# TaceoLabs/co-snarks

Hardware: AMD Instinct MI355X
Metric: BN254 G1 MSM points/sec (higher is better)
Workload: dtype i32x9 29-bit-limb lazy Montgomery, i64 accumulate (BN254 Fq 254-bit); 1 GPU; BN254 G1 Pippenger MSM, uniform scalars / known-dlog points, 2^20 points per GPU (BASELINE config 2); points_total=1048576, points_per_gpu=1048576, split=single GPU, exchange_mode=none, rccl_ranks_seen=0, spinup_steps=190

## Files before the change

### co-snarks_amd/csrc/msm_impl.hpp

```cpp
#pragma once
#include <stdlib.h>
#include <string.h>

#include <algorithm>
#include <type_traits>
#include <vector>

#include "common.hpp"
#include "curve.hpp"
#include "curve_lazy.hpp"
#include "curve_quad.hpp"
#include "curve_pair.hpp"
#include "host_fp64.hpp"
#include "msm_digits.hpp"
#include "msm_plan.hpp"
#include "msm_sort.hpp"
#include "msm_sort_wide.hpp"


namespace csh {

struct Bn254G1Cfg { using Fq = Bn254Fq;   using Fr = Bn254Fr; static constexpr bool LAZY = true;  using L = Fq29s; static constexpr bool INLINE_ADD = true; static constexpr bool PAIR = false; };
struct Bn254G2Cfg { using Fq = Bn254Fq2;  using Fr = Bn254Fr; static constexpr bool LAZY = true;  using L = Fq29s2; static constexpr bool INLINE_ADD = true; static constexpr bool PAIR = true; static constexpr bool PAIR_ACC_DEFAULT = false; using LP = Fp2Pair<Fq29s>; };
struct Bls381G1Cfg { using Fq = Bls381Fq;  using Fr = Bls381Fr; static constexpr bool LAZY = true;  using L = Fq28s; static constexpr bool INLINE_ADD = true; static constexpr bool PAIR = false; };
// ... 458 lines not shown
}

template <class Cfg, bool FUSED>
__global__ __launch_bounds__(RED_BLK) void k_msm_reduce_pair(MsmParams p, const LazyPt<Cfg>* __restrict__ dense, LazyPt<Cfg>* segres,
                                                             const uint32_t* __restrict__ start, const LazyPt<Cfg>* __restrict__ partial) {
  using L = typename Cfg::LP;
  const int w = blockIdx.y;
  const int role = pair_role();
  const uint32_t k = blockIdx.x * (RED_BLK / 2) + (threadIdx.x >> 1);
  if (k >= p.S) return;
  const uint32_t per = (p.NB + p.S - 1) / p.S;
  const uint32_t t0 = 1 + k * per;
  uint32_t t1 = t0 + per;
  if (t1 > p.NB + 1) t1 = p.NB + 1;
  XYZZLazy<L> running = XYZZLazy<L>::inf(), acc = XYZZLazy<L>::inf();
  uint32_t prev_b = 0;
  if (t0 < t1) {
    const LazyPt<Cfg>* dw = dense + (size_t)w * (p.NB + 1);
    const uint32_t* st = FUSED ? start + (size_t)w * (p.NB + 2) : nullptr;
    const LazyPt<Cfg>* pw = FUSED ? partial + (size_t)w * p.tmax : nullptr;
    for (uint32_t t = t1; t-- > t0;) {
      XYZZLazy<L> pt;
      if constexpr (FUSED) {
        pt = pbucket_merged<Cfg>(lane_len(p, w), st, pw, dw, t, role);
        if (pt.empty) continue;
      } else {
        if (dw[t].empty) continue;
        pt = pair_load(&dw[t], role);
      }
      uint32_t gap = prev_b ? prev_b - t : 0;
      if (gap) {
        if (gap <= 4) {
          while (gap--) lazy_add_inl<L>(acc, running);
        } else {
          const XYZZLazy<L> m = lazy_mul_small<L, true>(running, gap);
          lazy_add_inl<L>(acc, m);
        }
      }
      lazy_add_inl<L>(running, pt);
      prev_b = t;
    }
    if (prev_b) {
      const XYZZLazy<L> m = lazy_mul_small<L, true>(running, prev_b);
      lazy_add_inl<L>(acc, m);
    }
  }
  pair_store(&segres[(size_t)w * p.S + k], role, acc);
}

template <class Cfg>
__global__ __launch_bounds__(256) void k_msm_fold_tree(const LazyPt<Cfg>* __restrict__ in, uint32_t stride_in, uint32_t count,
                                                       LazyPt<Cfg>* out, uint32_t stride_out, XYZZ<typename Cfg::Fq>* win_out) {
  using L = typename Cfg::L;
  using Fq = typename Cfg::Fq;
  __shared__ XYZZLazy<L> sh[32];
  const int w = blockIdx.y;
  const int role = threadIdx.x & 3, q = threadIdx.x >> 2;
  const LazyPt<Cfg>* a = in + (size_t)w * stride_in;
  const uint32_t i0 = blockIdx.x * 128 + q, i1 = i0 + 64;
  QPt<L> x = i0 < count ? qpt_load<L>(&a[i0], role) : qpt_inf<L>();
  if (i1 < count) qadd<L>(x, qpt_load<L>(&a[i1], role), role);
  quad_block_tree<L>(x, sh, q, 64, role);
  if (q == 0) {
    if (win_out) {
      static_assert(sizeof(XYZZ<Fq>) == 4 * sizeof(Fq), "XYZZ members must be contiguous");
      (&win_out[w].x)[role] = x.empty ? Fq::zero() : x.v.to_fp();
    } else {
      qpt_store<L>(&out[(size_t)w * stride_out + blockIdx.x], role, x);
    }
  }
}

template <class Cfg>
__global__ __launch_bounds__(256) void k_bases_repack(Affine<typename Cfg::Fq>* pts, size_t n) {
  if constexpr (Cfg::LAZY) {
    using L = typename Cfg::L;
    for (size_t i = blockIdx.x * (size_t)256 + threadIdx.x; i < n; i += (size_t)gridDim.x * 256) {
      Affine<typename Cfg::Fq> p = pts[i];
      if (p.is_inf()) continue;
      p.x = L::repack_for_storage(p.x);
      p.y = L::repack_for_storage(p.y);
      pts[i] = p;
    }
  }
}

template <class Cfg>
__global__ void k_msm_gather_windows(const LazyPt<Cfg>* segres, uint32_t stride, int W, XYZZ<typename Cfg::Fq>* out) {
  const int w = threadIdx.x;
  if (w < W) out[w] = lazy_to_xyzz<typename Cfg::L, typename Cfg::Fq>(segres[(size_t)w * stride]);
}

extern thread_local float tl_msm_timing[6];
extern thread_local uint32_t tl_msm_params[4];
inline void msm_record_params(const MsmParams& srt) {
  tl_msm_params[0] = (uint32_t)srt.c;
  tl_msm_params[1] = (uint32_t)srt.W;
  tl_msm_params[2] = srt.L;
  tl_msm_params[3] = srt.S;
}

struct Events {
  std::vector<hipEvent_t> ev;
  Events() = default;
  Events(const Events&) = delete;
  Events& operator=(const Events&) = delete;
  ~Events() {
    for (hipEvent_t e : ev) (void)hipEventDestroy(e);
  }
  int create(size_t count, unsigned flags) {
    ev.reserve(ev.size() + count);
    for (size_t i = 0; i < count; ++i) {
      hipEvent_t e;
      CSH_HIP(hipEventCreateWithFlags(&e, flags));
      ev.push_back(e);
    }
    return CSH_OK;
  }
  hipEvent_t operator[](size_t i) const { return ev[i]; }
};

struct PartialHeader {
  uint32_t magic, c, W, wide;
  uint32_t pad[4];
};
constexpr uint32_t PARTIAL_MAGIC = 0x4d534d50u;


struct SortOut {
  uint32_t *start, *nlanes, *sorted;
};

inline bool msm_sort_is_wide(const MsmParams& p) { return p.c > 16 && p.W == 1 && p.remap_n != 0; }
template <class Fr>
constexpr int fr_id_of() {
  return std::is_same<Fr, Bls381Fr>::value ? 1 : (std::is_same<Fr, Bn254Fq>::value ? 2 : (std::is_same<Fr, Bls377Fr>::value ? 3 : 0));
}

struct SortStageBufs {
  SortBuffers sb;
  bool two_level;
};
inline SortBuffers sort_group_view(const MsmParams& p, const SortBuffers& b, int w0) {
  const size_t len = (size_t)p.NB + 2, n = p.n;
  SortBuffers g = b;
  g.hist += len * w0;
  g.start += len * w0;
  g.nlanes += w0;
  g.sorted += n * w0;
  g.dig += n * w0;
  g.blkcnt += (size_t)p.NB * p.CH * w0;
  if (g.inter) g.inter += n * w0;
  if (g.part_cnt) g.part_cnt += (size_t)(p.NB / 256) * p.CH * w0;
  return g;
}
inline SortStageBufs sort_take(const MsmParams& p, Arena& ar) {
  const size_t len = (size_t)p.NB + 2, n = p.n;
  SortStageBufs s;
  s.sb.hist = ar.take<uint32_t>(len * p.W);
  s.sb.start = ar.take<uint32_t>(len * p.W);
  s.sb.nlanes = ar.take<uint32_t>(MAX_WINDOWS);
  s.sb.sorted = ar.take<uint32_t>(n * p.W);
  s.sb.dig = ar.take<uint16_t>(n * p.W);
  s.sb.blkcnt = ar.take<uint32_t>((size_t)p.NB * p.CH * p.W);
  s.two_level = msm_sort_two_level(p);
  s.sb.inter = s.two_level ? ar.take<uint64_t>(n * p.W) : nullptr;
  s.sb.part_cnt = s.two_level ? ar.take<uint32_t>((size_t)(p.NB / 256) * p.CH * p.W) : nullptr;
  return s;
}
inline size_t msm_sort_bytes(const MsmParams& p, const MsmParams& pdig) {
  if (msm_sort_is_wide(p)) return msm_sort_wide_bytes(p, pdig);
  Arena sizing;
  sort_take(p, sizing);
  return sizing.off;
}
template <class Fr>
int msm_sort_prepare(const MsmParams& p, const MsmParams& pdig, const uint64_t* scalars_dev, hipStream_t st, Arena& ar, SortStageBufs* out) {
  *out = sort_take(p, ar);
  const int g1 = grid_for(pdig.n, MSM_BLK, 65536);
  hipLaunchKernelGGL(k_msm_digits<Fr>, dim3(g1), dim3(MSM_BLK), 0, st, reinterpret_cast<const Fr*>(scalars_dev), pdig, const_cast<uint16_t*>(out->sb.dig));
  return CSH_OK;
}
template <class Fr>
int msm_sort_stage(const MsmParams& p, const MsmParams& pdig, const uint64_t* scalars_dev, hipStream_t st, Arena& ar, SortOut* out, hipEvent_t* ev) {
  if (msm_sort_is_wide(p)) return msm_sort_wide_launch(fr_id_of<Fr>(), p, pdig, scalars_dev, st, ar, &out->start, &out->nlanes, &out->sorted, ev);
  SortStageBufs ss;
  CSH_TRY(msm_sort_prepare<Fr>(p, pdig, scalars_dev, st, ar, &ss));
  CSH_TRY(msm_sort_launch(p, ss.sb, st, ev));
  *out = SortOut{ss.sb.start, ss.sb.nlanes, ss.sb.sorted};
  return CSH_OK;
}

template <class Cfg>
struct BucketBufs {
  LazyPt<Cfg>*partial, *segres, *dense, *fold_a, *fold_b;
  uint32_t* giant;
  uint32_t* big;
  LazyPt<Cfg>* gscratch;
  uint32_t fold_n1, max_lanes, max_giant, giant_blocks;
};
constexpr int MAX_GROUPS = 8;
template <class Cfg>
BucketBufs<Cfg> bucket_take(const MsmParams& p, Arena& ar) {
  BucketBufs<Cfg> b;
  b.max_lanes = (uint32_t)(((size_t)p.n + p.L - 1) / p.L);
  b.max_giant = (uint32_t)(((uint64_t)b.max_lanes * p.W) / MERGE_CAP + 1);
  b.giant_blocks = b.max_giant < 1024 ? b.max_giant : 1024;
  b.partial = ar.take<LazyPt<Cfg>>((size_t)p.tmax * p.W);
  b.segres = ar.take<LazyPt<Cfg>>((size_t)p.S * p.W);
  b.dense = ar.take<LazyPt<Cfg>>((size_t)(p.NB + 1) * p.W);
  b.giant = ar.take<uint32_t>((2 * (size_t)b.max_giant + 2) * MAX_GROUPS);
  b.big = ar.take<uint32_t>((size_t)2 * GIANT_BIG_CAP * MAX_GROUPS);
  b.gscratch = ar.take<LazyPt<Cfg>>((size_t)GIANT_BIG_CAP * GIANT_SLICES * MAX_GROUPS);
  b.fold_n1 = (p.S + 127) / 128;
  b.fold_a = ar.take<LazyPt<Cfg>>((size_t)b.fold_n1 * p.W);
  b.fold_b = ar.take<LazyPt<Cfg>>((size_t)b.fold_n1 * p.W);
  return b;
}
template <class Cfg>
size_t msm_bucket_bytes(const MsmParams* pp) {
  Arena sizing;
  bucket_take<Cfg>(*pp, sizing);
  return sizing.off;
}

template <class Cfg>
struct BucketSumViews {
  const uint32_t *start, *nlanes, *sorted;
  LazyPt<Cfg>*partial, *dense;
  uint32_t *giant, *big;
  LazyPt<Cfg>* gscratch;
};
template <class Cfg>
int bucket_sums_launch(const Affine<typename Cfg::Fq>* bases, const MsmParams& p, const BucketSumViews<Cfg>& v, uint32_t max_lanes, uint32_t giant_blocks, int nw,
                       bool pair, bool fused, hipStream_t st, hipEvent_t* ev) {
  {
    const int tb = tune().acc_blk.load(std::memory_order_relaxed);
    const int blk = (tb == 64 || tb == 128) ? tb : ACC_BLK;
    if constexpr (Cfg::PAIR) {
      if (pair) {
        const dim3 ag((2 * max_lanes + blk - 1) / blk, nw), ab(blk);
        hipLaunchKernelGGL(k_msm_accum_pair<Cfg>, ag, ab, 0, st, bases, p, v.start, v.nlanes, v.sorted, v.partial, v.giant);
      }
    }
    if (!(Cfg::PAIR && pair)) {
      const dim3 ag((max_lanes + blk - 1) / blk, nw), ab(blk);
      hipLaunchKernelGGL(k_msm_accum<Cfg>, ag, ab, 0, st, bases, p, v.start, v.nlanes, v.sorted, v.partial, v.giant);
    }
  }
  if (ev) CSH_HIP(hipEventRecord(ev[4], st));
  if (fused)
    hipLaunchKernelGGL(k_msm_mark_giant<Cfg>, dim3((p.NB + 255) / 256, nw), dim3(256), 0, st, p, v.start, v.giant, v.giant + 2, v.big);
  else
    hipLaunchKernelGGL(k_msm_merge<Cfg>, dim3((p.NB + MERGE_Q - 1) / MERGE_Q, nw), dim3(MERGE_BLK), 0, st, p, v.start, v.partial, v.dense, v.giant, v.giant + 2, v.big);
  hipLaunchKernelGGL(k_msm_giant_slices<Cfg>, dim3(GIANT_SLICES, GIANT_ROWS), dim3(256), 0, st, p, v.start, v.partial, v.giant, v.big, v.gscratch);
  hipLaunchKernelGGL(k_msm_merge_giant<Cfg>, dim3(giant_blocks), dim3(256), 0, st, p, v.start, v.partial, v.dense, v.giant, v.giant + 2, v.big, v.gscratch);
  return CSH_OK;
}

template <class Cfg>
int bucket_group(const void* points, const MsmParams& p_all, const SortOut& so, const BucketBufs<Cfg>& bb, int w0, int nw, int group, hipStream_t st,
                 void* win_out_dev, hipEvent_t* ev) {
  using Fq = typename Cfg::Fq;
  MsmParams p = p_all;
  p.wide = p_all.wide > w0 ? p_all.wide - w0 : 0;
  const size_t len = (size_t)p.NB + 2;
  const uint32_t* start = so.start + len * w0;
  LazyPt<Cfg>* partial = bb.partial + (size_t)p.tmax * w0;
  LazyPt<Cfg>* segres = bb.segres + (size_t)p.S * w0;
  LazyPt<Cfg>* dense = bb.dense + (size_t)(p.NB + 1) * w0;
  LazyPt<Cfg>* fold_a = bb.fold_a + (size_t)bb.fold_n1 * w0;
  LazyPt<Cfg>* fold_b = bb.fold_b + (size_t)bb.fold_n1 * w0;
  const BucketSumViews<Cfg> views{start, so.nlanes + w0, so.sorted + (size_t)p.n * w0, partial, dense, bb.giant + (2 * (size_t)bb.max_giant + 2) * group,
                                  bb.big + (size_t)2 * GIANT_BIG_CAP * group, bb.gscratch + (size_t)GIANT_BIG_CAP * GIANT_SLICES * group};
  const int variant = tune().msm_variant.load(std::memory_order_relaxed);
  bool pair = false;
  if constexpr (Cfg::PAIR) pair = Cfg::PAIR_ACC_DEFAULT != ((variant & 2) != 0);
  int form;
  if constexpr (Cfg::PAIR) form = (variant & 1) ? 1 : ((variant & 4) ? 0 : 2);
  else form = (variant & 1) ? 0 : 1;
  const bool fused = form != 0 && (variant & 16) != 0;
  CSH_TRY((bucket_sums_launch<Cfg>(reinterpret_cast<const Affine<Fq>*>(points), p, views, bb.max_lanes, bb.giant_blocks, nw, pair, fused, st, ev)));
  MsmParams pr = p;
  if (form == 1) {
    pr.S = std::min(p.S, reduce_segments(p.NB, p.W, 4));
    if (fused) hipLaunchKernelGGL((k_msm_reduce<Cfg, true>), dim3((pr.S + 63) / 64, nw), dim3(256), 0, st, pr, dense, segres, start, partial);
    else hipLaunchKernelGGL((k_msm_reduce<Cfg, false>), dim3((pr.S + 63) / 64, nw), dim3(256), 0, st, pr, dense, segres, start, partial);
  } else if (form == 2) {
    pr.S = std::min(p.S, reduce_segments(p.NB, p.W, 2));
    if constexpr (Cfg::PAIR) {
      if (fused) hipLaunchKernelGGL((k_msm_reduce_pair<Cfg, true>), dim3((pr.S + RED_BLK / 2 - 1) / (RED_BLK / 2), nw), dim3(RED_BLK), 0, st, pr, dense, segres, start, partial);
      else hipLaunchKernelGGL((k_msm_reduce_pair<Cfg, false>), dim3((pr.S + RED_BLK / 2 - 1) / (RED_BLK / 2), nw), dim3(RED_BLK), 0, st, pr, dense, segres, start, partial);
    }
  } else {
    hipLaunchKernelGGL(k_msm_reduce_serial<Cfg>, dim3((pr.S + RED_BLK - 1) / RED_BLK, nw), dim3(RED_BLK), 0, st, pr, dense, segres);
  }
  const LazyPt<Cfg>* cur = segres;
  uint32_t cur_n = pr.S, cur_stride = pr.S;
  LazyPt<Cfg>* nxt = fold_a;
  XYZZ<Fq>* win_out = reinterpret_cast<XYZZ<Fq>*>(win_out_dev) + w0;
  bool exported = false;
  while (cur_n > 1) {
    const uint32_t out_n = (cur_n + 127) / 128;
    exported = out_n == 1;
    hipLaunchKernelGGL(k_msm_fold_tree<Cfg>, dim3(out_n, nw), dim3(256), 0, st, cur, cur_stride, cur_n, nxt, bb.fold_n1,
                       exported ? win_out : (XYZZ<Fq>*)nullptr);
    cur = nxt;
    cur_n = out_n;
    cur_stride = bb.fold_n1;
    nxt = nxt == fold_a ? fold_b : fold_a;
  }
  if (!exported)
    hipLaunchKernelGGL(k_msm_gather_windows<Cfg>, dim3(1), dim3(MAX_WINDOWS), 0, st, cur, cur_stride, nw, win_out);
  CSH_HIP(hipGetLastError());
  return CSH_OK;
}

template <class Cfg>
int msm_bucket_stage(const void* points, const MsmParams* pp, const SortOut* so, hipStream_t st, Arena* arp, void* win_out_dev, hipEvent_t* ev) {
  const MsmParams& p = *pp;
// ... 459 lines not shown
```

### co-snarks_amd/csrc/msm_sort.hip

```cpp
#include <stdlib.h>

#include "msm_sort.hpp"

namespace csh {

__device__ __forceinline__ uint32_t entry_id(const MsmParams& p, size_t i) {
  if (p.remap_n == 0) return (uint32_t)i;
  const uint32_t f = (uint32_t)i;
  const uint32_t w = f / p.remap_n;
  return w * p.remap_stride + p.remap_off + (f - w * p.remap_n);
}

__global__ __launch_bounds__(SORT_BLK) void k_msm_hist_lds(MsmParams p, const uint16_t* __restrict__ dig, uint32_t* __restrict__ blkcnt,
                                                            uint32_t* __restrict__ part_cnt ) {
  extern __shared__ uint32_t lds_cnt[];
  const uint32_t ch = blockIdx.x, w = blockIdx.y;
  for (uint32_t b = threadIdx.x; b < p.NB; b += SORT_BLK) lds_cnt[b] = 0;
  __syncthreads();
  const size_t lo = (size_t)ch * p.chunk_len;
  size_t hi = lo + p.chunk_len;
  if (hi > p.n) hi = p.n;
  const uint16_t* d = dig + (size_t)w * p.n;
  for (size_t i0 = lo; i0 < hi; i0 += 4 * SORT_BLK) {
    uint32_t code[4];
#pragma unroll
    for (int k = 0; k < 4; ++k) {
      const size_t i = i0 + (size_t)k * SORT_BLK + threadIdx.x;
      code[k] = i < hi ? (uint32_t)d[i] : DIG_ZERO;
    }
#pragma unroll
    for (int k = 0; k < 4; ++k) (void)lds_slot(lds_cnt, code[k] & 0x7fffu, code[k] != DIG_ZERO);
  }
  __syncthreads();
  uint32_t* out = blkcnt + ((size_t)w * p.CH + ch) * p.NB;
  for (uint32_t b = threadIdx.x; b < p.NB; b += SORT_BLK) out[b] = lds_cnt[b];
  if (part_cnt) {
    const uint32_t P = p.NB / 256;
    const int lane = threadIdx.x & 63;
    for (uint32_t part = threadIdx.x >> 6; part < P; part += SORT_BLK / 64) {
      const uint32_t* c = lds_cnt + part * 256;
      uint32_t v = c[lane] + c[lane + 64] + c[lane + 128] + c[lane + 192];
#pragma unroll
      for (int d = 32; d >= 1; d >>= 1) v += (uint32_t)__shfl_xor((int)v, d);
      if (lane == 0) part_cnt[((size_t)w * p.CH + ch) * P + part] = v;
    }
  }
}

__global__ __launch_bounds__(256) void k_msm_colscan(MsmParams p, uint32_t* __restrict__ blkcnt, uint32_t* __restrict__ hist) {
  const uint32_t w = blockIdx.y;
  const uint32_t b = blockIdx.x * 256 + threadIdx.x;
  if (b >= p.NB) return;
  uint32_t acc = 0;
  uint32_t* col = blkcnt + (size_t)w * p.CH * p.NB + b;
  for (uint32_t ch0 = 0; ch0 < p.CH; ch0 += 8) {
    uint32_t t[8];
#pragma unroll
    for (uint32_t j = 0; j < 8; ++j) t[j] = ch0 + j < p.CH ? col[(size_t)(ch0 + j) * p.NB] : 0u;
#pragma unroll
    for (uint32_t j = 0; j < 8; ++j) {
      if (ch0 + j < p.CH) col[(size_t)(ch0 + j) * p.NB] = acc;
      acc += t[j];
    }
  }
  hist[(size_t)w * (p.NB + 2) + b + 1] = acc;
  if (b == 0) {
    hist[(size_t)w * (p.NB + 2)] = 0;
    hist[(size_t)w * (p.NB + 2) + p.NB + 1] = 0;
  }
}

__global__ __launch_bounds__(1024) void k_msm_scan(MsmParams p, uint32_t* hist, uint32_t* start, uint32_t* nlanes) {
  extern __shared__ uint32_t sc_lds[];
  const int w = blockIdx.x;
  const uint32_t len = p.NB + 2;
  uint32_t* h = hist + (size_t)w * len;
  uint32_t* st = start + (size_t)w * len;
  uint32_t* wave_tot = sc_lds + len;
  for (uint32_t b = threadIdx.x; b < len; b += 1024) sc_lds[b] = h[b];
  __syncthreads();
  const uint32_t per = (len + 1023) / 1024;
  const uint32_t b0 = threadIdx.x * per;
  uint32_t cnt = 0;
  for (uint32_t k = 0; k < per; ++k) {
    const uint32_t b = b0 + k;
    if (b < len) cnt += sc_lds[b];
  }
  uint32_t total;
  uint32_t run_c = block_excl_scan<16>(cnt, wave_tot, &total);
  for (uint32_t k = 0; k < per; ++k) {
    const uint32_t b = b0 + k;
    if (b < len) {
      const uint32_t cv = sc_lds[b];
      sc_lds[b] = run_c;
      run_c += cv;
    }
  }
  __syncthreads();
  for (uint32_t b = threadIdx.x; b < len; b += 1024) {
    st[b] = sc_lds[b];
    h[b] = sc_lds[b];
  }
  if (threadIdx.x == 0) nlanes[w] = (total + lane_len(p, w) - 1) / lane_len(p, w);
}

__global__ __launch_bounds__(SORT_BLK) void k_msm_scatter_lds(MsmParams p, const uint16_t* __restrict__ dig,
                                                               const uint32_t* __restrict__ start, const uint32_t* __restrict__ blkcnt,
                                                               uint32_t* __restrict__ sorted) {
  extern __shared__ uint32_t lds_cur[];
  const uint32_t ch = blockIdx.x, w = blockIdx.y;
  const uint32_t* st = start + (size_t)w * (p.NB + 2) + 1;
  const uint32_t* pre = blkcnt + ((size_t)w * p.CH + ch) * p.NB;
  for (uint32_t b = threadIdx.x; b < p.NB; b += SORT_BLK) lds_cur[b] = st[b] + pre[b];
  __syncthreads();
  const size_t lo = (size_t)ch * p.chunk_len;
  size_t hi = lo + p.chunk_len;
  if (hi > p.n) hi = p.n;
  const uint16_t* d = dig + (size_t)w * p.n;
  uint32_t* so = sorted + (size_t)w * p.n;
  for (size_t i0 = lo; i0 < hi; i0 += SORT_BLK) {
    const size_t i = i0 + threadIdx.x;
    uint32_t code = DIG_ZERO;
    if (i < hi) code = d[i];
    const bool valid = code != DIG_ZERO;
    const uint32_t pos = lds_slot(lds_cur, code & 0x7fffu, valid);
    if (valid) so[pos] = entry_id(p, i) | ((code >> 15) << 31);
  }
}


constexpr uint32_t PART_BUCKETS = 256;
constexpr uint32_t PART_LB = 8;
static_assert(PART_BUCKETS == 1u << PART_LB, "the record format's low key must hold a partition's bucket index");

__global__ __launch_bounds__(256) void k_msm_part_offsets(MsmParams p, const uint32_t* __restrict__ start, uint32_t* part_cnt) {
  const uint32_t P = p.NB / PART_BUCKETS;
  const uint32_t part = blockIdx.x * 256 + threadIdx.x, w = blockIdx.y;
  if (part >= P) return;
  uint32_t run = start[(size_t)w * (p.NB + 2) + (size_t)part * PART_BUCKETS + 1];
  uint32_t* col = part_cnt + (size_t)w * p.CH * P + part;
  for (uint32_t ch0 = 0; ch0 < p.CH; ch0 += 8) {
    uint32_t c[8];
#pragma unroll
    for (uint32_t j = 0; j < 8; ++j) c[j] = ch0 + j < p.CH ? col[(size_t)(ch0 + j) * P] : 0u;
#pragma unroll
    for (uint32_t j = 0; j < 8; ++j) {
      if (ch0 + j < p.CH) col[(size_t)(ch0 + j) * P] = run;
      run += c[j];
    }
  }
}

#ifndef CSH_L1_WPE
#define CSH_L1_WPE 8
#endif
#if CSH_L1_WPE > 0
#define CSH_L1_OCC __attribute__((amdgpu_waves_per_eu(CSH_L1_WPE)))
#else
#define CSH_L1_OCC
#endif
constexpr int L1_EPT = 8;
constexpr int L1_TILE = L1_EPT * SORT_BLK;
constexpr uint32_t MAXP = 128;
template <int REC>
__global__ __launch_bounds__(SORT_BLK) CSH_L1_OCC void k_msm_scatter_l1(MsmParams p, const uint16_t* __restrict__ dig, const uint32_t* __restrict__ part_off,
                                                             void* __restrict__ inter) {
  __shared__ uint32_t gcur[MAXP];
  __shared__ uint32_t cnt[MAXP];
  __shared__ uint32_t toff[MAXP];
  __shared__ uint32_t wsum[2];
  __shared__ uint32_t pay[L1_TILE];
  __shared__ uint8_t slo[L1_TILE];
  __shared__ uint8_t sbin[L1_TILE];
  const uint32_t ch = blockIdx.x, w = blockIdx.y, tid = threadIdx.x;
  const uint32_t P = p.NB / PART_BUCKETS;
  if (tid < MAXP) {
    gcur[tid] = tid < P ? part_off[((size_t)w * p.CH + ch) * P + tid] : 0;
    cnt[tid] = 0;
  }
  __syncthreads();
  const size_t lo = (size_t)ch * p.chunk_len;
  size_t hi = lo + p.chunk_len;
  if (hi > p.n) hi = p.n;
  const uint16_t* d = dig + (size_t)w * p.n;
  SortRec<REC>* out = reinterpret_cast<SortRec<REC>*>(inter) + (size_t)w * p.n;
  for (size_t t0 = lo; t0 < hi; t0 += L1_TILE) {
    uint32_t code[L1_EPT], rank[L1_EPT];
#pragma unroll
    for (int k = 0; k < L1_EPT; ++k) {
      const size_t i = t0 + (size_t)k * SORT_BLK + tid;
      code[k] = i < hi ? (uint32_t)__builtin_nontemporal_load(d + i) : DIG_ZERO;
    }
#pragma unroll
    for (int k = 0; k < L1_EPT; ++k) rank[k] = lds_slot(cnt, (code[k] & 0x7fffu) / PART_BUCKETS, code[k] != DIG_ZERO);
    __syncthreads();
    const uint32_t v = tid < MAXP ? cnt[tid] : 0;
    uint32_t tile_n;
    const uint32_t excl = block_excl_scan<MAXP / 64, SORT_BLK / 64>(v, wsum, &tile_n);
    if (tid < MAXP) toff[tid] = excl;
    __syncthreads();
#pragma unroll
    for (int k = 0; k < L1_EPT; ++k) {
      if (code[k] != DIG_ZERO) {
        const uint32_t b0 = code[k] & 0x7fffu;
        const uint32_t slot = toff[b0 / PART_BUCKETS] + rank[k];
        pay[slot] = entry_id(p, t0 + (size_t)k * SORT_BLK + tid) | ((code[k] >> 15) << 31);
        slo[slot] = (uint8_t)(b0 % PART_BUCKETS);
        sbin[slot] = (uint8_t)(b0 / PART_BUCKETS);
      }
    }
    __syncthreads();
#pragma unroll
    for (int k = 0; k < L1_EPT; ++k) {
      const uint32_t sl = k * SORT_BLK + tid;
      if (sl < tile_n) {
        const uint32_t bin = sbin[sl];
        out[gcur[bin] + (sl - toff[bin])] = rec_pack<REC>(pay[sl], slo[sl], PART_LB);
      }
    }
    __syncthreads();
    if (tid < MAXP) {
      gcur[tid] += v;
      cnt[tid] = 0;
    }
    __syncthreads();
  }
}

struct L2Lds {
  uint32_t obase[PART_BUCKETS];
  uint32_t cnt[PART_BUCKETS];
  uint32_t toff[PART_BUCKETS];
  uint32_t wsum[4];
  uint32_t pay[L2_TILE];
  uint8_t sbin[L2_TILE];
};
struct L2OwnRuns {
  __device__ void reserve(uint32_t*, uint32_t, uint32_t) const {}
  __device__ void advance(uint32_t* obase, uint32_t b, uint32_t v) const { obase[b] += v; }
};
struct L2SharedRuns {
  uint32_t* cur;
  __device__ void reserve(uint32_t* obase, uint32_t b, uint32_t v) const { obase[b] = v ? atomicAdd(&cur[b], v) : 0u; }
  __device__ void advance(uint32_t*, uint32_t, uint32_t) const {}
};
template <int REC, class Runs>
__device__ __forceinline__ void l2_sort_slice(L2Lds& s, const Runs runs, const SortRec<REC>* __restrict__ in, uint32_t lo, uint32_t hi,
                                              uint32_t* __restrict__ so) {
  const uint32_t tid = threadIdx.x;
  for (uint32_t t0 = lo; t0 < hi; t0 += L2_TILE) {
    SortRec<REC> e[L2_EPT];
    uint32_t rank[L2_EPT];
    l2_load_rank<REC>(in, t0, hi, PART_LB, s.cnt, e, rank);
    __syncthreads();
    uint32_t v = 0, total;
    if (tid < PART_BUCKETS) {
      v = s.cnt[tid];
      runs.reserve(s.obase, tid, v);
    }
    const uint32_t excl = block_excl_scan<PART_BUCKETS / 64, SORT_BLK / 64>(v, s.wsum, &total);
    if (tid < PART_BUCKETS) s.toff[tid] = excl;
    __syncthreads();
#pragma unroll
    for (int k = 0; k < L2_EPT; ++k) {
      if (t0 + k * SORT_BLK + tid < hi) {
        const uint32_t bin = rec_low<REC>(e[k], PART_LB);
        const uint32_t slot = s.toff[bin] + rank[k];
        s.pay[slot] = rec_entry<REC>(e[k], PART_LB);
        s.sbin[slot] = (uint8_t)bin;
      }
    }
    __syncthreads();
    const uint32_t tile_n = hi - t0 < (uint32_t)L2_TILE ? hi - t0 : (uint32_t)L2_TILE;
#pragma unroll
    for (int k = 0; k < L2_EPT; ++k) {
      const uint32_t sl = k * SORT_BLK + tid;
      if (sl < tile_n) {
        const uint32_t bin = s.sbin[sl];
        so[s.obase[bin] + (sl - s.toff[bin])] = s.pay[sl];
      }
    }
    __syncthreads();
    if (tid < PART_BUCKETS) {
      runs.advance(s.obase, tid, v);
      s.cnt[tid] = 0;
    }
    __syncthreads();
  }
}

template <int REC>
__global__ __launch_bounds__(SORT_BLK) void k_msm_scatter_l2(MsmParams p, const uint32_t* __restrict__ start, const void* __restrict__ inter,
                                                             uint32_t* __restrict__ sorted) {
  __shared__ L2Lds s;
  const uint32_t part = blockIdx.x, w = blockIdx.y, tid = threadIdx.x;
  const uint32_t* st = start + (size_t)w * (p.NB + 2) + (size_t)part * PART_BUCKETS + 1;
  if (tid < PART_BUCKETS) {
    s.obase[tid] = st[tid];
    s.cnt[tid] = 0;
  }
  __syncthreads();
  l2_sort_slice<REC>(s, L2OwnRuns{}, reinterpret_cast<const SortRec<REC>*>(inter) + (size_t)w * p.n, st[0], st[PART_BUCKETS],
                     sorted + (size_t)w * p.n);
}

template <int REC>
__global__ __launch_bounds__(SORT_BLK) void k_msm_scatter_l2t(MsmParams p, const uint32_t* __restrict__ start, uint32_t* __restrict__ cursor,
                                                              const void* __restrict__ inter, uint32_t* __restrict__ sorted) {
  __shared__ L2Lds s;
  __shared__ uint32_t job[3];
  const uint32_t x = blockIdx.x, w = blockIdx.y, tid = threadIdx.x;
  const uint32_t P = p.NB / PART_BUCKETS;
  const uint32_t* stw = start + (size_t)w * (p.NB + 2);
  {
    uint32_t lo_p = 0, hi_p = 0, nb = 0, total;
    if (tid < P) {
      lo_p = stw[(size_t)tid * PART_BUCKETS + 1];
      hi_p = stw[(size_t)(tid + 1) * PART_BUCKETS + 1];
      const uint32_t c = hi_p - lo_p;
      nb = c ? (c + L2_TILE / 2) / L2_TILE : 0;
      if (c && nb == 0) nb = 1;
    }
    if (tid == 0) job[0] = 0xffffffffu;
    const uint32_t pre = block_excl_scan<MAXP / 64, SORT_BLK / 64>(nb, s.wsum, &total);
    if (nb && x >= pre && x < pre + nb) {
      const uint32_t c = hi_p - lo_p, slice = (c + nb - 1) / nb, j = x - pre;
      uint32_t a = lo_p + j * slice, b = a + slice;
      if (b > hi_p) b = hi_p;
      if (a > hi_p) a = hi_p;
      job[0] = tid;
      job[1] = a;
      job[2] = b;
    }
    __syncthreads();
  }
  const uint32_t part = job[0];
  if (part == 0xffffffffu) return;
  if (tid < PART_BUCKETS) s.cnt[tid] = 0;
  __syncthreads();
  l2_sort_slice<REC>(s, L2SharedRuns{cursor + (size_t)w * (p.NB + 2) + (size_t)part * PART_BUCKETS + 1},
                     reinterpret_cast<const SortRec<REC>*>(inter) + (size_t)w * p.n, job[1], job[2], sorted + (size_t)w * p.n);
}

bool msm_sort_two_level(const MsmParams& p) {
  if (p.NB < 4 * PART_BUCKETS) return false;
  if (const int f = tune().sort_two_level.load(std::memory_order_relaxed); f >= 0) return f != 0;
  return p.n >= (1u << 20);
}

SortPath msm_sort_path(const MsmParams& p) {
  SortPath s{msm_sort_two_level(p), false, false};
  if (!s.two_level) return s;
  const uint64_t max_id = p.remap_n ? (uint64_t)(p.n / p.remap_n) * p.remap_stride : (uint64_t)p.n;
  const int variant = tune().msm_variant.load(std::memory_order_relaxed);
  s.rec4 = (variant & 8) == 0 && max_id <= (1u << (31 - PART_LB));
  s.per_partition = (variant & 32) != 0;
  return s;
}

template <int REC>
static void launch_two_level(const MsmParams& p, const SortBuffers& b, bool per_partition, hipStream_t st) {
  const uint32_t nparts = p.NB / PART_BUCKETS;
  hipLaunchKernelGGL(k_msm_scatter_l1<REC>, dim3(p.CH, p.W), dim3(SORT_BLK), 0, st, p, b.dig, b.part_cnt, (void*)b.inter);
  if (per_partition) {
    hipLaunchKernelGGL(k_msm_scatter_l2<REC>, dim3(nparts, p.W), dim3(SORT_BLK), 0, st, p, b.start, (const void*)b.inter, b.sorted);
  } else {
    const uint32_t l2_blocks = (uint32_t)(p.n / L2_TILE) + nparts + 1;
    hipLaunchKernelGGL(k_msm_scatter_l2t<REC>, dim3(l2_blocks, p.W), dim3(SORT_BLK), 0, st, p, b.start, b.hist, (const void*)b.inter, b.sorted);
  }
}

int msm_sort_launch(const MsmParams& p, const SortBuffers& b, hipStream_t st, hipEvent_t* ev) {
  const SortPath path = msm_sort_path(p);
  const bool two_level = path.two_level;
  const size_t sort_lds = sizeof(uint32_t) * p.NB;
  if (sort_lds > 48 * 1024) {
    CSH_TRY(raise_lds_limit((const void*)k_msm_hist_lds, 128 * 1024));
    CSH_TRY(raise_lds_limit((const void*)k_msm_scatter_lds, 128 * 1024));
  }
  hipLaunchKernelGGL(k_msm_hist_lds, dim3(p.CH, p.W), dim3(SORT_BLK), sort_lds, st, p, b.dig, b.blkcnt, two_level ? b.part_cnt : nullptr);
  hipLaunchKernelGGL(k_msm_colscan, dim3((p.NB + 255) / 256, p.W), dim3(256), 0, st, p, b.blkcnt, b.hist);
  if (ev) CSH_HIP(hipEventRecord(ev[1], st));
  {
    const size_t scan_lds = sizeof(uint32_t) * ((size_t)p.NB + 2 + 16);
    if (scan_lds > 48 * 1024) CSH_TRY(raise_lds_limit((const void*)k_msm_scan, 136 * 1024));
    hipLaunchKernelGGL(k_msm_scan, dim3(p.W), dim3(1024), scan_lds, st, p, b.hist, b.start, b.nlanes);
  }
  if (ev) CSH_HIP(hipEventRecord(ev[2], st));
  if (two_level) {
    hipLaunchKernelGGL(k_msm_part_offsets, dim3((p.NB / PART_BUCKETS + 255) / 256, p.W), dim3(256), 0, st, p, b.start, b.part_cnt);
    path.rec4 ? launch_two_level<1>(p, b, path.per_partition, st) : launch_two_level<0>(p, b, path.per_partition, st);
  } else {
    hipLaunchKernelGGL(k_msm_scatter_lds, dim3(p.CH, p.W), dim3(SORT_BLK), sort_lds, st, p, b.dig, b.start, b.blkcnt, b.sorted);
  }
  if (ev) CSH_HIP(hipEventRecord(ev[3], st));
  return CSH_OK;
}

}
```

### co-snarks_amd/csrc/msm_sort.hpp

```cpp
#pragma once
#include <type_traits>

#include "common.hpp"

namespace csh {

struct MsmParams {
  uint32_t n;
  int c;
  int W;
  uint32_t NB;
  uint32_t L;
  uint32_t tmax;
  uint32_t S;
  int mont;
  uint32_t CH;
  uint32_t chunk_len;
  uint32_t remap_n, remap_stride, remap_off;
  uint32_t dig_g, dig_wp;
  int wide;
  uint32_t Ln;
};
__host__ __device__ inline uint32_t lane_len(const MsmParams& p, int w) { return w >= p.wide ? p.Ln : p.L; }

constexpr uint32_t DIG_ZERO = 0xFFFFu;
constexpr int MAX_WINDOWS = 128;

struct SortBuffers {
  uint32_t* hist;
  uint32_t* start;
  uint32_t* nlanes;
  uint32_t* sorted;
  const uint16_t* dig;
  uint32_t* blkcnt;
  uint64_t* inter;
  uint32_t* part_cnt;
};

#if defined(__HIPCC__)
__device__ __forceinline__ uint32_t lds_slot(uint32_t* counter, uint32_t b, bool valid) {
  uint32_t slot = 0;
  bool todo = valid;
  for (int round = 0; round < 4; ++round) {
    const unsigned long long act = __ballot(todo);
    if (!act) return slot;
    const int leader = __ffsll((long long)act) - 1;
    const uint32_t lb = (uint32_t)__shfl((int)b, leader);
    const unsigned long long grp = __ballot(todo && b == lb);
    const int cnt = __popcll(grp);
    if (cnt < 8) break;
    uint32_t base = 0;
    const int lane = threadIdx.x & 63;
    if (lane == leader) base = atomicAdd(&counter[lb], (uint32_t)cnt);
    base = (uint32_t)__shfl((int)base, leader);
    if (todo && b == lb) {
      slot = base + (uint32_t)__popcll(grp & ((1ull << lane) - 1ull));
      todo = false;
    }
  }
  if (todo) slot = atomicAdd(&counter[b], 1u);
  return slot;
}

__device__ __forceinline__ uint32_t wave_incl_scan(uint32_t v) {
  const int lane = threadIdx.x & 63;
#pragma unroll
  for (int d = 1; d < 64; d <<= 1) {
    const uint32_t up = (uint32_t)__shfl_up((int)v, d);
    if (lane >= d) v += up;
  }
  return v;
}

template <int NW, int BLOCK_WAVES = NW>
__device__ __forceinline__ uint32_t block_excl_scan(uint32_t v, uint32_t* wsum, uint32_t* total) {
  const int lane = threadIdx.x & 63, wv = threadIdx.x >> 6;
  uint32_t incl = 0;
  if (BLOCK_WAVES == NW || wv < NW) {
    incl = wave_incl_scan(v);
    if (lane == 63) wsum[wv] = incl;
  }
  __syncthreads();
  uint32_t base = 0, tot = 0;
#pragma unroll
  for (int i = 0; i < NW; ++i) {
    const uint32_t t = wsum[i];
    if (i < wv) base += t;
    tot += t;
  }
  *total = tot;
  return base + incl - v;
}

template <int REC>
using SortRec = typename std::conditional<REC != 0, uint32_t, uint64_t>::type;
template <int REC>
__device__ __forceinline__ SortRec<REC> rec_pack(uint32_t entry, uint32_t low, uint32_t lb) {
  if constexpr (REC == 1) {
    const uint32_t idb = 31 - lb;
    return (entry & ((1u << idb) - 1)) | ((entry >> 31) << idb) | (low << (idb + 1));
  } else {
    return (uint64_t)entry | ((uint64_t)low << 32);
  }
}
template <int REC>
__device__ __forceinline__ uint32_t rec_low(SortRec<REC> e, uint32_t lb) {
  if constexpr (REC == 1) return e >> (32 - lb);
  else return (uint32_t)(e >> 32);
}
template <int REC>
__device__ __forceinline__ uint32_t rec_entry(SortRec<REC> e, uint32_t lb) {
  if constexpr (REC == 1) {
    const uint32_t idb = 31 - lb;
    return (e & ((1u << idb) - 1)) | (((e >> idb) & 1u) << 31);
  } else {
    return (uint32_t)e;
  }
}

constexpr int SORT_BLK = 1024;
constexpr int L2_EPT = 8;
constexpr int L2_TILE = L2_EPT * SORT_BLK;
template <int REC>
__device__ __forceinline__ void l2_load_rank(const SortRec<REC>* __restrict__ in, uint32_t t0, uint32_t hi, uint32_t lb, uint32_t* cnt,
                                             SortRec<REC>* e, uint32_t* rank) {
#pragma unroll
  for (int k = 0; k < L2_EPT; ++k) {
    const uint32_t i = t0 + k * SORT_BLK + threadIdx.x;
    e[k] = i < hi ? __builtin_nontemporal_load(in + i) : 0;
  }
#pragma unroll
  for (int k = 0; k < L2_EPT; ++k) rank[k] = lds_slot(cnt, rec_low<REC>(e[k], lb), t0 + k * SORT_BLK + threadIdx.x < hi);
}
#endif

bool msm_sort_two_level(const MsmParams& p);
struct SortPath {
  bool two_level;
  bool rec4;
  bool per_partition;
};
SortPath msm_sort_path(const MsmParams& p);
int msm_sort_launch(const MsmParams& p, const SortBuffers& b, hipStream_t st, hipEvent_t* ev);

}
```

Measured before the change: 663.9 million points/s.

## Precompute L2 sort jobs, prefetch L1 digit tiles, skip unused colscan prefix writes

Several sort-stage changes land together. The per-block job assignment that every L2 scatter block recomputed with a scan is moved into k_msm_part_offsets, which writes a job table once per window. The L1 scatter now does vectorized 4-digit loads, packs two ranks per register, and prefetches the next tile while the current one is scattered, and it merges the cursor updates to drop two barriers per tile. Colscan skips writing per-chunk prefixes when the two-level path does not use them. The cost is extra job-table memory, a single-block-per-window part_offsets kernel, and the prefetch registers may reduce occupancy.

```diff
diff --git a/co-snarks_amd/csrc/msm_impl.hpp b/co-snarks_amd/csrc/msm_impl.hpp
--- a/co-snarks_amd/csrc/msm_impl.hpp
+++ b/co-snarks_amd/csrc/msm_impl.hpp
@@ -634,6 +634,7 @@
   g.blkcnt += (size_t)p.NB * p.CH * w0;
   if (g.inter) g.inter += n * w0;
   if (g.part_cnt) g.part_cnt += (size_t)(p.NB / 256) * p.CH * w0;
+  if (g.l2_jobs) g.l2_jobs += (size_t)4 * msm_l2_jobs(p) * w0;
   return g;
 }
 inline SortStageBufs sort_take(const MsmParams& p, Arena& ar) {
@@ -648,6 +649,7 @@
   s.two_level = msm_sort_two_level(p);
   s.sb.inter = s.two_level ? ar.take<uint64_t>(n * p.W) : nullptr;
   s.sb.part_cnt = s.two_level ? ar.take<uint32_t>((size_t)(p.NB / 256) * p.CH * p.W) : nullptr;
+  s.sb.l2_jobs = s.two_level ? ar.take<uint32_t>((size_t)4 * msm_l2_jobs(p) * p.W) : nullptr;
   return s;
 }
 inline size_t msm_sort_bytes(const MsmParams& p, const MsmParams& pdig) {
diff --git a/co-snarks_amd/csrc/msm_sort.hip b/co-snarks_amd/csrc/msm_sort.hip
--- a/co-snarks_amd/csrc/msm_sort.hip
+++ b/co-snarks_amd/csrc/msm_sort.hip
@@ -47,6 +47,7 @@
   }
 }
 
+template <bool PREFIX>
 __global__ __launch_bounds__(256) void k_msm_colscan(MsmParams p, uint32_t* __restrict__ blkcnt, uint32_t* __restrict__ hist) {
   const uint32_t w = blockIdx.y;
   const uint32_t b = blockIdx.x * 256 + threadIdx.x;
@@ -59,7 +60,7 @@
     for (uint32_t j = 0; j < 8; ++j) t[j] = ch0 + j < p.CH ? col[(size_t)(ch0 + j) * p.NB] : 0u;
 #pragma unroll
     for (uint32_t j = 0; j < 8; ++j) {
-      if (ch0 + j < p.CH) col[(size_t)(ch0 + j) * p.NB] = acc;
+      if (PREFIX && ch0 + j < p.CH) col[(size_t)(ch0 + j) * p.NB] = acc;
       acc += t[j];
     }
   }
@@ -133,21 +134,60 @@
 constexpr uint32_t PART_LB = 8;
 static_assert(PART_BUCKETS == 1u << PART_LB, "the record format's low key must hold a partition's bucket index");
 
-__global__ __launch_bounds__(256) void k_msm_part_offsets(MsmParams p, const uint32_t* __restrict__ start, uint32_t* part_cnt) {
+constexpr uint32_t MAXP = 128;
+constexpr uint32_t L2_NO_JOB = 0xffffffffu;
+__global__ __launch_bounds__(256) void k_msm_part_offsets(MsmParams p, const uint32_t* __restrict__ start, uint32_t* part_cnt, uint4* __restrict__ jobs,
+                                                          uint32_t njobs) {
+  __shared__ uint32_t s_pre[MAXP + 1], s_lo[MAXP], s_hi[MAXP], s_wsum[4];
   const uint32_t P = p.NB / PART_BUCKETS;
-  const uint32_t part = blockIdx.x * 256 + threadIdx.x, w = blockIdx.y;
-  if (part >= P) return;
-  uint32_t run = start[(size_t)w * (p.NB + 2) + (size_t)part * PART_BUCKETS + 1];
-  uint32_t* col = part_cnt + (size_t)w * p.CH * P + part;
-  for (uint32_t ch0 = 0; ch0 < p.CH; ch0 += 8) {
-    uint32_t c[8];
-#pragma unroll
-    for (uint32_t j = 0; j < 8; ++j) c[j] = ch0 + j < p.CH ? col[(size_t)(ch0 + j) * P] : 0u;
-#pragma unroll
-    for (uint32_t j = 0; j < 8; ++j) {
-      if (ch0 + j < p.CH) col[(size_t)(ch0 + j) * P] = run;
-      run += c[j];
-    }
+  const uint32_t part = threadIdx.x, w = blockIdx.x;
+  uint32_t lo_p = 0, hi_p = 0;
+  if (part < P) {
+    lo_p = start[(size_t)w * (p.NB + 2) + (size_t)part * PART_BUCKETS + 1];
+    hi_p = start[(size_t)w * (p.NB + 2) + (size_t)(part + 1) * PART_BUCKETS + 1];
+    uint32_t run = lo_p;
+    uint32_t* col = part_cnt + (size_t)w * p.CH * P + part;
+    for (uint32_t ch0 = 0; ch0 < p.CH; ch0 += 8) {
+      uint32_t c[8];
+#pragma unroll
+      for (uint32_t j = 0; j < 8; ++j) c[j] = ch0 + j < p.CH ? col[(size_t)(ch0 + j) * P] : 0u;
+#pragma unroll
+      for (uint32_t j = 0; j < 8; ++j) {
+        if (ch0 + j < p.CH) col[(size_t)(ch0 + j) * P] = run;
+        run += c[j];
+      }
+    }
+  }
+  if (!jobs) return;
+  const uint32_t c = hi_p - lo_p;
+  uint32_t nb = c ? (c + L2_TILE / 2) / L2_TILE : 0;
+  if (c && nb == 0) nb = 1;
+  uint32_t total;
+  const uint32_t pre = block_excl_scan<4>(nb, s_wsum, &total);
+  if (part < MAXP) {
+    s_pre[part] = pre;
+    s_lo[part] = lo_p;
+    s_hi[part] = hi_p;
+  }
+  if (part == 0) s_pre[MAXP] = total;
+  __syncthreads();
+  uint4* jw = jobs + (size_t)w * njobs;
+  for (uint32_t x = threadIdx.x; x < njobs; x += 256) {
+    uint4 job = make_uint4(L2_NO_JOB, 0, 0, 0);
+    if (x < total) {
+      uint32_t a = 0, b = MAXP;
+      while (b - a > 1) {
+        const uint32_t mid = (a + b) >> 1;
+        if (s_pre[mid] <= x) a = mid; else b = mid;
+      }
+      const uint32_t q = a, lo_q = s_lo[q], hi_q = s_hi[q], cq = hi_q - lo_q, nq = s_pre[q + 1] - s_pre[q];
+      const uint32_t slice = (cq + nq - 1) / nq, j = x - s_pre[q];
+      uint32_t first = lo_q + j * slice, last = first + slice;
+      if (last > hi_q) last = hi_q;
+      if (first > hi_q) first = hi_q;
+      job = make_uint4(q, first, last, 0);
+    }
+    jw[x] = job;
   }
 }
 
@@ -159,52 +199,86 @@
 #else
 #define CSH_L1_OCC
 #endif
-constexpr int L1_EPT = 8;
+#ifndef CSH_L1_GROUPS
+#define CSH_L1_GROUPS 2
+#endif
+constexpr int L1_GROUPS = CSH_L1_GROUPS;
+constexpr int L1_EPT = 4 * L1_GROUPS;
 constexpr int L1_TILE = L1_EPT * SORT_BLK;
-constexpr uint32_t MAXP = 128;
+constexpr int L1_PIECE = 4 * SORT_BLK;
+static_assert(L1_TILE <= (1 << 16), "two ranks inside the tile share one register");
+static_assert(2 * (6 * L1_TILE + 4096) <= 160 * 1024, "two blocks per CU");
+typedef uint32_t l1_group_t __attribute__((ext_vector_type(2)));
+__device__ __forceinline__ void l1_load_tile(const uint16_t* __restrict__ db, uint32_t e0, uint32_t last4, l1_group_t* c) {
+#pragma unroll
+  for (int j = 0; j < L1_GROUPS; ++j) {
+    const uint32_t e = e0 + (uint32_t)j * L1_PIECE + 4 * threadIdx.x;
+    c[j] = __builtin_nontemporal_load(reinterpret_cast<const l1_group_t*>(db + (e < last4 ? e : last4)));
+  }
+}
+__device__ __forceinline__ uint32_t l1_code(const l1_group_t* c, int k) { return (c[k / 4][(k / 2) & 1] >> (16 * (k & 1))) & 0xffffu; }
 template <int REC>
 __global__ __launch_bounds__(SORT_BLK) CSH_L1_OCC void k_msm_scatter_l1(MsmParams p, const uint16_t* __restrict__ dig, const uint32_t* __restrict__ part_off,
                                                              void* __restrict__ inter) {
-  __shared__ uint32_t gcur[MAXP];
   __shared__ uint32_t cnt[MAXP];
   __shared__ uint32_t toff[MAXP];
+  __shared__ uint32_t gbase[MAXP];
   __shared__ uint32_t wsum[2];
   __shared__ uint32_t pay[L1_TILE];
   __shared__ uint8_t slo[L1_TILE];
   __shared__ uint8_t sbin[L1_TILE];
   const uint32_t ch = blockIdx.x, w = blockIdx.y, tid = threadIdx.x;
   const uint32_t P = p.NB / PART_BUCKETS;
+  const uint32_t lo = ch * p.chunk_len;
+  const uint32_t hi = p.n - lo < p.chunk_len ? p.n : lo + p.chunk_len;
+  if (lo >= p.n) return;
+  uint32_t gcur = 0;
   if (tid < MAXP) {
-    gcur[tid] = tid < P ? part_off[((size_t)w * p.CH + ch) * P + tid] : 0;
+    gcur = tid < P ? part_off[((size_t)w * p.CH + ch) * P + tid] : 0;
     cnt[tid] = 0;
   }
   __syncthreads();
-  const size_t lo = (size_t)ch * p.chunk_len;
-  size_t hi = lo + p.chunk_len;
-  if (hi > p.n) hi = p.n;
-  const uint16_t* d = dig + (size_t)w * p.n;
+  const size_t row = (size_t)w * p.n;
+  const uint32_t r = (uint32_t)(row & 3);
+  const uint16_t* db = dig + (row - r);
+  const uint32_t last4 = (r + hi - 1) & ~3u;
   SortRec<REC>* out = reinterpret_cast<SortRec<REC>*>(inter) + (size_t)w * p.n;
-  for (size_t t0 = lo; t0 < hi; t0 += L1_TILE) {
-    uint32_t code[L1_EPT], rank[L1_EPT];
+  l1_group_t code[L1_GROUPS];
+  l1_load_tile(db, (r + lo) & ~3u, last4, code);
+  for (uint32_t e0 = (r + lo) & ~3u; e0 < r + hi; e0 += L1_TILE) {
+    const uint32_t i0 = e0 + 4 * tid - r;
+    uint32_t rank[L1_EPT / 2];
 #pragma unroll
     for (int k = 0; k < L1_EPT; ++k) {
-      const size_t i = t0 + (size_t)k * SORT_BLK + tid;
-      code[k] = i < hi ? (uint32_t)__builtin_nontemporal_load(d + i) : DIG_ZERO;
-    }
-#pragma unroll
-    for (int k = 0; k < L1_EPT; ++k) rank[k] = lds_slot(cnt, (code[k] & 0x7fffu) / PART_BUCKETS, code[k] != DIG_ZERO);
-    __syncthreads();
-    const uint32_t v = tid < MAXP ? cnt[tid] : 0;
+      const uint32_t i = i0 + (uint32_t)(k / 4) * L1_PIECE + (k % 4);
+      if (i - lo >= hi - lo) code[k / 4][(k / 2) & 1] |= 0xffffu << (16 * (k & 1));
+      const uint32_t c = l1_code(code, k);
+      const uint32_t rk = lds_slot(cnt, (c & 0x7fffu) / PART_BUCKETS, c != DIG_ZERO);
+      rank[k / 2] = (k & 1) ? rank[k / 2] | (rk << 16) : rk;
+    }
+    __syncthreads();
+    l1_group_t nxt[L1_GROUPS];
+    l1_load_tile(db, e0 + L1_TILE, last4, nxt);
+    uint32_t v = 0;
+    if (tid < MAXP) {
+      v = cnt[tid];
+      cnt[tid] = 0;
+    }
     uint32_t tile_n;
     const uint32_t excl = block_excl_scan<MAXP / 64, SORT_BLK / 64>(v, wsum, &tile_n);
-    if (tid < MAXP) toff[tid] = excl;
+    if (tid < MAXP) {
+      toff[tid] = excl;
+      gbase[tid] = gcur - excl;
+      gcur += v;
+    }
     __syncthreads();
 #pragma unroll
     for (int k = 0; k < L1_EPT; ++k) {
-      if (code[k] != DIG_ZERO) {
-        const uint32_t b0 = code[k] & 0x7fffu;
-        const uint32_t slot = toff[b0 / PART_BUCKETS] + rank[k];
-        pay[slot] = entry_id(p, t0 + (size_t)k * SORT_BLK + tid) | ((code[k] >> 15) << 31);
+      const uint32_t c = l1_code(code, k);
+      if (c != DIG_ZERO) {
+        const uint32_t b0 = c & 0x7fffu;
+        const uint32_t slot = toff[b0 / PART_BUCKETS] + ((rank[k / 2] >> (16 * (k & 1))) & 0xffffu);
+        pay[slot] = entry_id(p, i0 + (uint32_t)(k / 4) * L1_PIECE + (k % 4)) | ((c >> 15) << 31);
         slo[slot] = (uint8_t)(b0 % PART_BUCKETS);
         sbin[slot] = (uint8_t)(b0 / PART_BUCKETS);
       }
@@ -213,17 +287,10 @@
 #pragma unroll
     for (int k = 0; k < L1_EPT; ++k) {
       const uint32_t sl = k * SORT_BLK + tid;
-      if (sl < tile_n) {
-        const uint32_t bin = sbin[sl];
-        out[gcur[bin] + (sl - toff[bin])] = rec_pack<REC>(pay[sl], slo[sl], PART_LB);
-      }
-    }
-    __syncthreads();
-    if (tid < MAXP) {
-      gcur[tid] += v;
-      cnt[tid] = 0;
-    }
-    __syncthreads();
+      if (sl < tile_n) out[gbase[sbin[sl]] + sl] = rec_pack<REC>(pay[sl], slo[sl], PART_LB);
+    }
+#pragma unroll
+    for (int j = 0; j < L1_GROUPS; ++j) code[j] = nxt[j];
   }
 }
 
@@ -236,12 +303,14 @@
   uint8_t sbin[L2_TILE];
 };
 struct L2OwnRuns {
-  __device__ void reserve(uint32_t*, uint32_t, uint32_t) const {}
+  __device__ uint32_t reserve(uint32_t, uint32_t) const { return 0; }
+  __device__ void publish(uint32_t*, uint32_t, uint32_t) const {}
   __device__ void advance(uint32_t* obase, uint32_t b, uint32_t v) const { obase[b] += v; }
 };
 struct L2SharedRuns {
   uint32_t* cur;
-  __device__ void reserve(uint32_t* obase, uint32_t b, uint32_t v) const { obase[b] = v ? atomicAdd(&cur[b], v) : 0u; }
+  __device__ uint32_t reserve(uint32_t b, uint32_t v) const { return v ? atomicAdd(&cur[b], v) : 0u; }
+  __device__ void publish(uint32_t* obase, uint32_t b, uint32_t first) const { obase[b] = first; }
   __device__ void advance(uint32_t*, uint32_t, uint32_t) const {}
 };
 template <int REC, class Runs>
@@ -253,10 +322,10 @@
     uint32_t rank[L2_EPT];
     l2_load_rank<REC>(in, t0, hi, PART_LB, s.cnt, e, rank);
     __syncthreads();
-    uint32_t v = 0, total;
+    uint32_t v = 0, first = 0, total;
     if (tid < PART_BUCKETS) {
       v = s.cnt[tid];
-      runs.reserve(s.obase, tid, v);
+      first = runs.reserve(tid, v);
     }
     const uint32_t excl = block_excl_scan<PART_BUCKETS / 64, SORT_BLK / 64>(v, s.wsum, &total);
     if (tid < PART_BUCKETS) s.toff[tid] = excl;
@@ -270,6 +339,7 @@
         s.sbin[slot] = (uint8_t)bin;
       }
     }
+    if (tid < PART_BUCKETS) runs.publish(s.obase, tid, first);
     __syncthreads();
     const uint32_t tile_n = hi - t0 < (uint32_t)L2_TILE ? hi - t0 : (uint32_t)L2_TILE;
 #pragma unroll
@@ -305,41 +375,16 @@
 }
 
 template <int REC>
-__global__ __launch_bounds__(SORT_BLK) void k_msm_scatter_l2t(MsmParams p, const uint32_t* __restrict__ start, uint32_t* __restrict__ cursor,
+__global__ __launch_bounds__(SORT_BLK) void k_msm_scatter_l2t(MsmParams p, const uint4* __restrict__ jobs, uint32_t* __restrict__ cursor,
                                                               const void* __restrict__ inter, uint32_t* __restrict__ sorted) {
   __shared__ L2Lds s;
-  __shared__ uint32_t job[3];
-  const uint32_t x = blockIdx.x, w = blockIdx.y, tid = threadIdx.x;
-  const uint32_t P = p.NB / PART_BUCKETS;
-  const uint32_t* stw = start + (size_t)w * (p.NB + 2);
-  {
-    uint32_t lo_p = 0, hi_p = 0, nb = 0, total;
-    if (tid < P) {
-      lo_p = stw[(size_t)tid * PART_BUCKETS + 1];
-      hi_p = stw[(size_t)(tid + 1) * PART_BUCKETS + 1];
-      const uint32_t c = hi_p - lo_p;
-      nb = c ? (c + L2_TILE / 2) / L2_TILE : 0;
-      if (c && nb == 0) nb = 1;
-    }
-    if (tid == 0) job[0] = 0xffffffffu;
-    const uint32_t pre = block_excl_scan<MAXP / 64, SORT_BLK / 64>(nb, s.wsum, &total);
-    if (nb && x >= pre && x < pre + nb) {
-      const uint32_t c = hi_p - lo_p, slice = (c + nb - 1) / nb, j = x - pre;
-      uint32_t a = lo_p + j * slice, b = a + slice;
-      if (b > hi_p) b = hi_p;
-      if (a > hi_p) a = hi_p;
-      job[0] = tid;
-      job[1] = a;
-      job[2] = b;
-    }
-    __syncthreads();
-  }
-  const uint32_t part = job[0];
-  if (part == 0xffffffffu) return;
+  const uint32_t w = blockIdx.y, tid = threadIdx.x;
+  const uint4 job = jobs[(size_t)w * gridDim.x + blockIdx.x];
+  if (job.x == L2_NO_JOB) return;
   if (tid < PART_BUCKETS) s.cnt[tid] = 0;
   __syncthreads();
-  l2_sort_slice<REC>(s, L2SharedRuns{cursor + (size_t)w * (p.NB + 2) + (size_t)part * PART_BUCKETS + 1},
-                     reinterpret_cast<const SortRec<REC>*>(inter) + (size_t)w * p.n, job[1], job[2], sorted + (size_t)w * p.n);
+  l2_sort_slice<REC>(s, L2SharedRuns{cursor + (size_t)w * (p.NB + 2) + (size_t)job.x * PART_BUCKETS + 1},
+                     reinterpret_cast<const SortRec<REC>*>(inter) + (size_t)w * p.n, job.y, job.z, sorted + (size_t)w * p.n);
 }
 
 bool msm_sort_two_level(const MsmParams& p) {
@@ -365,8 +410,8 @@
   if (per_partition) {
     hipLaunchKernelGGL(k_msm_scatter_l2<REC>, dim3(nparts, p.W), dim3(SORT_BLK), 0, st, p, b.start, (const void*)b.inter, b.sorted);
   } else {
-    const uint32_t l2_blocks = (uint32_t)(p.n / L2_TILE) + nparts + 1;
-    hipLaunchKernelGGL(k_msm_scatter_l2t<REC>, dim3(l2_blocks, p.W), dim3(SORT_BLK), 0, st, p, b.start, b.hist, (const void*)b.inter, b.sorted);
+    hipLaunchKernelGGL(k_msm_scatter_l2t<REC>, dim3(msm_l2_jobs(p), p.W), dim3(SORT_BLK), 0, st, p, reinterpret_cast<const uint4*>(b.l2_jobs), b.hist,
+                       (const void*)b.inter, b.sorted);
   }
 }
 
@@ -379,7 +424,9 @@
     CSH_TRY(raise_lds_limit((const void*)k_msm_scatter_lds, 128 * 1024));
   }
   hipLaunchKernelGGL(k_msm_hist_lds, dim3(p.CH, p.W), dim3(SORT_BLK), sort_lds, st, p, b.dig, b.blkcnt, two_level ? b.part_cnt : nullptr);
-  hipLaunchKernelGGL(k_msm_colscan, dim3((p.NB + 255) / 256, p.W), dim3(256), 0, st, p, b.blkcnt, b.hist);
+  const dim3 colscan_grid((p.NB + 255) / 256, p.W);
+  if (two_level) hipLaunchKernelGGL(k_msm_colscan<false>, colscan_grid, dim3(256), 0, st, p, b.blkcnt, b.hist);
+  else hipLaunchKernelGGL(k_msm_colscan<true>, colscan_grid, dim3(256), 0, st, p, b.blkcnt, b.hist);
   if (ev) CSH_HIP(hipEventRecord(ev[1], st));
   {
     const size_t scan_lds = sizeof(uint32_t) * ((size_t)p.NB + 2 + 16);
@@ -388,7 +435,9 @@
   }
   if (ev) CSH_HIP(hipEventRecord(ev[2], st));
   if (two_level) {
-    hipLaunchKernelGGL(k_msm_part_offsets, dim3((p.NB / PART_BUCKETS + 255) / 256, p.W), dim3(256), 0, st, p, b.start, b.part_cnt);
+    static_assert(MAXP <= 256, "k_msm_part_offsets: one thread per partition of a window");
+    hipLaunchKernelGGL(k_msm_part_offsets, dim3(p.W), dim3(256), 0, st, p, b.start, b.part_cnt,
+                       path.per_partition ? nullptr : reinterpret_cast<uint4*>(b.l2_jobs), msm_l2_jobs(p));
     path.rec4 ? launch_two_level<1>(p, b, path.per_partition, st) : launch_two_level<0>(p, b, path.per_partition, st);
   } else {
     hipLaunchKernelGGL(k_msm_scatter_lds, dim3(p.CH, p.W), dim3(SORT_BLK), sort_lds, st, p, b.dig, b.start, b.blkcnt, b.sorted);
diff --git a/co-snarks_amd/csrc/msm_sort.hpp b/co-snarks_amd/csrc/msm_sort.hpp
--- a/co-snarks_amd/csrc/msm_sort.hpp
+++ b/co-snarks_amd/csrc/msm_sort.hpp
@@ -35,6 +35,7 @@
   uint32_t* blkcnt;
   uint64_t* inter;
   uint32_t* part_cnt;
+  uint32_t* l2_jobs;
 };
 
 #if defined(__HIPCC__)
@@ -121,6 +122,7 @@
 constexpr int SORT_BLK = 1024;
 constexpr int L2_EPT = 8;
 constexpr int L2_TILE = L2_EPT * SORT_BLK;
+inline uint32_t msm_l2_jobs(const MsmParams& p) { return p.n / L2_TILE + p.NB / 256 + 1; }
 template <int REC>
 __device__ __forceinline__ void l2_load_rank(const SortRec<REC>* __restrict__ in, uint32_t t0, uint32_t hi, uint32_t lb, uint32_t* cnt,
                                              SortRec<REC>* e, uint32_t* rank) {
```

New measurement: 647.0 million points/s. 2.5% lower.
